# PKU-VCL-Geometry/GeoSplatting

Measured on AMD Instinct MI355X. Metric: fwd+bwd views/sec at 2M Gaussians, 800x800, higher is better.
Workload: dtype f32

## Files before the change

geosplatting_amd/csrc/gs_front.hip:

```cpp
#include "gs_common.h"
#include <string.h>
#pragma clang fp contract(off)
#include "gs_project_dev.h"
#include "gs_shade_dev.h"

template <int CTRL, int ROW_MASK>
__device__ __forceinline__ unsigned dpp_max_u32(unsigned v)
{
    const unsigned o = (unsigned)__builtin_amdgcn_update_dpp(0, (int)v, CTRL, ROW_MASK, 0xf, false);
    return o > v ? o : v;
}
__device__ __forceinline__ unsigned wave_max_u32_lane63(unsigned v)
{
    v = dpp_max_u32<0xB1, 0xf>(v);
    v = dpp_max_u32<0x4E, 0xf>(v);
    v = dpp_max_u32<0x141, 0xf>(v);
    v = dpp_max_u32<0x140, 0xf>(v);
    v = dpp_max_u32<0x142, 0xa>(v);
    v = dpp_max_u32<0x143, 0xc>(v);
    return v;
}

__global__ void __launch_bounds__(GS_PROJ_BLOCK)
front_fwd_kernel(int N, const float* __restrict__ means, const float* __restrict__ quats, const float* __restrict__ scales,
                 const float* __restrict__ opacities, const float* __restrict__ normals, const float* __restrict__ kd,
                 const float* __restrict__ ks, const float* __restrict__ viewmat, const float* __restrict__ K,
                 const float* __restrict__ cam_pos, float min_roughness, float max_metallic, int mode, EnvDev env,
                 int W, int H, int tile_size, int tile_w, int tile_h, float eps2d, float near_plane, float far_plane, float radius_clip,
                 unsigned key_base, unsigned key_limit , float4* __restrict__ vis, unsigned* __restrict__ depth_keys,
                 uint2* __restrict__ rects, unsigned* __restrict__ ctrl, u64* __restrict__ desc, int n_chunks,
                 unsigned long long* __restrict__ counts , long long* __restrict__ status,
                 unsigned* __restrict__ tile_counts , int32_t* __restrict__ packed_index ,
                 int tight_tiles)
{
    extern __shared__ unsigned s_th[];
    const int n_tiles = tile_w * tile_h;
    if (tile_counts) for (int t = threadIdx.x; t < n_tiles; t += GS_PROJ_BLOCK) s_th[t] = 0u;
    __shared__ int s_chunk;
    __shared__ int s_wv[GS_PROJ_WAVES];
    __shared__ int s_wi[GS_PROJ_WAVES];
    __shared__ unsigned s_wmx[GS_PROJ_WAVES], s_wmn[GS_PROJ_WAVES];
    __shared__ long long s_base[2];

    const int tid = threadIdx.x, lane = tid & 63, wave = tid >> 6;
    if (tid == 0) s_chunk = (int)atomicAdd(ctrl, 1u);
    __syncthreads();
    const int chunk = s_chunk;
    const int n = chunk * GS_PROJ_BLOCK + tid;

    u64* agg_v = desc;
    u64* agg_i = desc + n_chunks;
    u64* pre_v = desc + 2 * (size_t)n_chunks;
    u64* pre_i = desc + 3 * (size_t)n_chunks;

    const GsCam cam = load_cam(viewmat, K);
    ProjFwd p;
    p.valid = false; p.radius = 0;
    int ntiles = 0;
    int tx0 = 0, ty0 = 0, tx1 = 0, ty1 = 0;
    float mean[3] = { 0.f, 0.f, 0.f };
    float op = 0.0f, hx = -1.0f, hy = -1.0f;
    if (n < N) {
        mean[0] = means[3 * (size_t)n]; mean[1] = means[3 * (size_t)n + 1]; mean[2] = means[3 * (size_t)n + 2];
        const float4 q = *reinterpret_cast<const float4*>(quats + 4 * (size_t)n);
        const float quat[4] = { q.x, q.y, q.z, q.w };
        const float scale[3] = { scales[3 * (size_t)n], scales[3 * (size_t)n + 1], scales[3 * (size_t)n + 2] };
        p = project_exact(cam, mean, quat, scale, (float)W, (float)H, eps2d, near_plane, far_plane, radius_clip);
        if (p.valid) {
            tile_range_exact(p.m2x, p.m2y, p.radius, tile_size, tile_w, tile_h, tx0, ty0, tx1, ty1);
            op = opacities[n] * p.comp;
            if (!alpha_extent(p.ca, p.cb, p.cc, op, hx, hy)) { hx = -1.0f; hy = -1.0f; }
            if (tight_tiles) {
                if (hx < 0.0f) { tx1 = tx0; ty1 = ty0; }
                else {
                    const float ts = (float)tile_size;
                    const float fx0 = floorf((p.m2x - hx) / ts), fy0 = floorf((p.m2y - hy) / ts);
                    const float fx1 = ceilf((p.m2x + hx) / ts), fy1 = ceilf((p.m2y + hy) / ts);
                    const int ax0 = fx0 < 0.0f ? 0 : (fx0 > (float)tile_w ? tile_w : (int)fx0), ax1 = fx1 < 0.0f ? 0 : (fx1 > (float)tile_w ? tile_w : (int)fx1);
                    const int ay0 = fy0 < 0.0f ? 0 : (fy0 > (float)tile_h ? tile_h : (int)fy0), ay1 = fy1 < 0.0f ? 0 : (fy1 > (float)tile_h ? tile_h : (int)fy1);
                    tx0 = max(tx0, ax0); tx1 = min(tx1, ax1); ty0 = max(ty0, ay0); ty1 = min(ty1, ay1);
                    if (tx1 < tx0) tx1 = tx0;
                    if (ty1 < ty0) ty1 = ty0;
                }
            }
            ntiles = (tx1 - tx0) * (ty1 - ty0);
        }
    }

    const u64 bal = __ballot(p.valid);
    const int v_excl_wave = __popcll(bal & ((1ull << lane) - 1ull));
    int i_incl = ntiles;
    i_incl = gs_wave_incl_scan(i_incl);
    const unsigned dbits = p.valid ? __float_as_uint(p.depth) : 0u;
    {
        const unsigned mx = wave_max_u32_lane63(dbits), mn = wave_max_u32_lane63(p.valid ? ~dbits : 0u);
        if (lane == 63) { s_wv[wave] = __popcll(bal); s_wi[wave] = i_incl; s_wmx[wave] = mx; s_wmn[wave] = mn; }
    }
    __syncthreads();
    int v_before = 0, i_before = 0, aggV = 0, aggI = 0;
#pragma unroll
    for (int w = 0; w < GS_PROJ_WAVES; ++w) {
        if (w < wave) { v_before += s_wv[w]; i_before += s_wi[w]; }
        aggV += s_wv[w]; aggI += s_wi[w];
    }
    if (wave == 0 && lane == 0 && chunk > 0) { desc_store(&agg_v[chunk], (u64)aggV); desc_store(&agg_i[chunk], (u64)aggI); }

    const bool range_wave = wave == GS_PROJ_WAVES - 1;
    unsigned long long cur_mx = 0ull, cur_mn = 0ull;
    if (range_wave && lane == 0 && aggV != 0) {
        cur_mx = __hip_atomic_load(counts + 3, __ATOMIC_RELAXED, __HIP_MEMORY_SCOPE_AGENT);
        cur_mn = __hip_atomic_load(counts + 2, __ATOMIC_RELAXED, __HIP_MEMORY_SCOPE_AGENT);
    }

    float color[3] = { 0.f, 0.f, 0.f };
    if (p.valid && vis != nullptr) {
        const float nrm[3] = { normals[3 * (size_t)n], normals[3 * (size_t)n + 1], normals[3 * (size_t)n + 2] };
        const float kdn[3] = { kd[3 * (size_t)n], kd[3 * (size_t)n + 1], kd[3 * (size_t)n + 2] };
        const float2 ks2 = *reinterpret_cast<const float2*>(ks + 2 * (size_t)n);
        const float ksn[2] = { ks2.x, ks2.y };
        const float cp[3] = { cam_pos[0], cam_pos[1], cam_pos[2] };
        ShadeTmp t;
        shade_one<false>(mean, nrm, kdn, ksn, cp, min_roughness, max_metallic, mode, env, color, t);
    }
    if (range_wave && lane == 0 && aggV != 0) {
        unsigned mx = 0u, mn = 0u;
#pragma unroll
        for (int w = 0; w < GS_PROJ_WAVES; ++w) { mx = s_wmx[w] > mx ? s_wmx[w] : mx; mn = s_wmn[w] > mn ? s_wmn[w] : mn; }
        if ((unsigned long long)mx > cur_mx) atomicMax(counts + 3, (unsigned long long)mx);
        if ((unsigned long long)mn > cur_mn) atomicMax(counts + 2, (unsigned long long)mn);
    }
    unsigned key = dbits;
    if (key_limit != 0u) {
        const bool fits = dbits >= key_base && (dbits - key_base) < key_limit;
        if (p.valid && !fits && status) status[3] = 1;
        key = fits ? dbits - key_base : (dbits < key_base ? 0u : key_limit - 1u);
    }

    if (wave == 0) {
        long long baseV = 0, baseI = 0;
        if (chunk > 0) {
            int pos = chunk - 1;
            for (;;) {
                const int idx = pos - lane;
                bool isP = idx < 0;
                bool isA = false;
                u64 pv = 0, pi = 0, av = 0, ai = 0;
                if (idx >= 0) {
                    int spins = 0;
                    for (;;) {
                        pv = desc_load(&pre_v[idx]); pi = desc_load(&pre_i[idx]);
                        isP = (pv & pi & GS_VALID_BIT) != 0;
                        if (isP) break;
                        av = desc_load(&agg_v[idx]); ai = desc_load(&agg_i[idx]);
                        isA = (av & ai & GS_VALID_BIT) != 0;
                        if (isA) break;
                        if (++spins > GS_SPIN_LIMIT) {
                            atomicExch(ctrl + 1, 1u);
                            if (status) status[0] = GS_ENOSPC;
                            isA = true; av = ai = 0; break;
                        }
                        __builtin_amdgcn_s_sleep(2);
                    }
                }
                const u64 pmask = __ballot(isP);
                const int first = pmask ? __builtin_ctzll(pmask) : 64;
                long long cv = 0, ci = 0;
                if (lane <= first) {
                    cv = (long long)((isP ? pv : av) & ~GS_VALID_BIT);
                    ci = (long long)((isP ? pi : ai) & ~GS_VALID_BIT);
                }
                baseV += wave_sum_i64(cv);
                baseI += wave_sum_i64(ci);
                if (pmask) break;
                pos -= 64;
            }
        }
        if (lane == 0) {
            desc_store(&pre_i[chunk], (u64)(baseI + aggI));
            desc_store(&pre_v[chunk], (u64)(baseV + aggV));
            s_base[0] = baseV; s_base[1] = baseI;
            if (chunk == n_chunks - 1) { counts[0] = (unsigned long long)(baseV + aggV); counts[1] = (unsigned long long)(baseI + aggI); }
        }
    }
    __syncthreads();
    if (packed_index && n < N) packed_index[n] = p.valid ? (int32_t)(s_base[0] + v_before + v_excl_wave) : -1;
    if (p.valid) {
        const long long slot = s_base[0] + v_before + v_excl_wave;
        if (vis != nullptr) {
            float4* rec = vis + 4 * slot;
            rec[0] = make_float4(p.m2x, p.m2y, 0.5f * p.ca, p.cb);
            rec[1] = make_float4(0.5f * p.cc, op, hx, hy);
            rec[2] = make_float4(color[0], color[1], color[2], 0.0f);
            rec[3] = make_float4(p.comp, __int_as_float(n), p.depth, __int_as_float(p.radius));
        }
        if (depth_keys != nullptr) {
            depth_keys[slot] = key;
            rects[slot] = make_uint2((unsigned)tx0 | ((unsigned)ty0 << 16), (unsigned)tx1 | ((unsigned)ty1 << 16));
        }
        if (tile_counts)
            for (int i = ty0; i < ty1; ++i)
                for (int j = tx0; j < tx1; ++j) atomicAdd(&s_th[i * tile_w + j], 1u);
    }
    if (tile_counts) {
        __syncthreads();
        for (int t = threadIdx.x; t < n_tiles; t += GS_PROJ_BLOCK) { const unsigned c = s_th[t]; if (c) atomicAdd(tile_counts + t, c); }
    }
}

__global__ void __launch_bounds__(256)
front_setup_kernel(unsigned* __restrict__ ws, int ws_words, unsigned long long* __restrict__ counts4, unsigned* __restrict__ tile_counts, int n_tiles)
{
    const int i = blockIdx.x * blockDim.x + threadIdx.x, stride = gridDim.x * blockDim.x;
    for (int k = i; k < ws_words; k += stride) ws[k] = 0u;
    for (int k = i; k < n_tiles; k += stride) tile_counts[k] = 0u;
    if (i < 4) counts4[i] = 0ull;
}

#define GS_FRONT_HIST_MAX 8192
extern "C" size_t gs_front_ws_bytes(int N) { return (gs_project_ws_bytes(N) + 15) & ~(size_t)15; }

extern "C" int gs_front_fwd(int N, const float* means, const float* quats, const float* scales, const float* opacities,
                            const float* normals, const float* kd, const float* ks, const float* viewmat, const float* K,
                            const float* cam_pos, float min_roughness, float max_metallic, int mode, const GsEnv* env,
                            int W, int H, int tile_size, float eps2d, float near_plane, float far_plane, float radius_clip,
                            uint32_t key_base, int key_bits, float* vis_records, uint32_t* depth_keys, uint32_t* tile_rects,
                            uint32_t* tile_counts, int32_t* packed_index, int tight_tiles, int64_t* counts4, int64_t* status4, void* ws,
                            size_t ws_bytes, void* stream)
{
    GS_CHECK_ARG(N >= 0 && W > 0 && H > 0 && tile_size > 0 && mode >= 0 && mode <= 2, "bad sizes or mode");
    GS_CHECK_ARG(counts4 != nullptr && ws != nullptr, "null argument");
    GS_CHECK_ARG((depth_keys != nullptr) == (tile_rects != nullptr) && (vis_records != nullptr || depth_keys != nullptr),
                 "depth_keys and tile_rects go together; at least one of {vis_records} / {depth_keys, tile_rects} is wanted");
    GS_CHECK_ARG(key_bits == 24 || key_bits == 32, "key_bits must be 24 or 32");
    GS_CHECK_ARG(key_bits == 32 || status4 != nullptr, "24-bit keys need a status word (range overflow is reported there)");
    EnvDev e;
    if (vis_records != nullptr) GS_CHECK_ARG(env_to_dev(env, e) == 0, "bad GsEnv");
    else memset(&e, 0, sizeof(e));
    if (ws_bytes < gs_front_ws_bytes(N)) { gs_set_error("gs_front_fwd: workspace too small"); return GS_ENOSPC; }
    hipStream_t s = (hipStream_t)stream;
    const int tile_w = (W + tile_size - 1) / tile_size, tile_h = (H + tile_size - 1) / tile_size;
    GS_CHECK_ARG(tile_w < 65536 && tile_h < 65536, "tile grid too large");
    const int n_tiles = tile_w * tile_h;
    const bool hist = tile_counts != nullptr && n_tiles <= GS_FRONT_HIST_MAX;
    const int ws_words = (int)(gs_front_ws_bytes(N) / 4);
    hipLaunchKernelGGL(front_setup_kernel, dim3(gs_cdiv(ws_words > n_tiles ? ws_words : n_tiles, 256) < 64 ? gs_cdiv(ws_words > n_tiles ? ws_words : n_tiles, 256) : 64),
                       dim3(256), 0, s, (unsigned*)ws, ws_words, (unsigned long long*)counts4, tile_counts, tile_counts ? n_tiles : 0);
    GS_CHECK_LAUNCH();
    if (N == 0) return GS_OK;
    const int n_chunks = (N + GS_PROJ_BLOCK - 1) / GS_PROJ_BLOCK;
    hipLaunchKernelGGL(front_fwd_kernel, dim3(n_chunks), dim3(GS_PROJ_BLOCK), hist ? (size_t)n_tiles * sizeof(unsigned) : 0, s, N, means, quats, scales, opacities, normals, kd, ks,
                       viewmat, K, cam_pos, min_roughness, max_metallic, mode, e, W, H, tile_size, tile_w, tile_h, eps2d, near_plane,
                       far_plane, radius_clip, key_bits == 24 ? key_base : 0u, key_bits == 24 ? (1u << 24) : 0u, (float4*)vis_records,
                       depth_keys, (uint2*)tile_rects, (unsigned*)ws, (u64*)((char*)ws + 16), n_chunks, (unsigned long long*)counts4,
                       (long long*)status4, hist ? tile_counts : (unsigned*)nullptr, packed_index, tight_tiles);
    GS_CHECK_LAUNCH();
    return GS_OK;
}

template <int BLOCK>
__global__ void __launch_bounds__(BLOCK)
tail_bwd_kernel(GsCount vc, const float* __restrict__ means, const float* __restrict__ quats, const float* __restrict__ scales,
                const float* __restrict__ opacities, const float* __restrict__ normals, const float* __restrict__ kd,
                const float* __restrict__ ks, const float* __restrict__ viewmat, const float* __restrict__ K,
                const float* __restrict__ cam_pos, float min_roughness, float max_metallic, int mode, EnvDev env, int W, int H,
                float eps2d, const float4* __restrict__ vis, const float* __restrict__ v_packed, int rec_stride,
                float* __restrict__ v_means, float* __restrict__ v_quats, float* __restrict__ v_scales, float* __restrict__ v_opacities,
                float* __restrict__ v_normals, float* __restrict__ v_kd, float* __restrict__ v_ks, EnvGradDev eg)
{
    extern __shared__ __attribute__((aligned(16))) float s_grad[];
    for (int i = threadIdx.x; i < eg.lds_floats; i += blockDim.x) s_grad[i] = 0.0f;
    __syncthreads();
    float* const stage = s_grad + eg.stage_off + (threadIdx.x >> 6) * 640;
    float* const priv = eg.priv ? eg.priv + (long long)gs_xcc_id() * eg.priv_stride : nullptr;
    const float cp[3] = { cam_pos[0], cam_pos[1], cam_pos[2] };
    const GsCam cam = load_cam(viewmat, K);
    const int V = (int)gs_count(vc);
    const int stride = (int)(gridDim.x * blockDim.x);
    const int n_iter = (V + stride - 1) / stride;
    for (int it = 0; it < n_iter; ++it) {
        const int v = it * stride + blockIdx.x * blockDim.x + threadIdx.x;
        bool scatter = false;
        ShadeTmp t;
        float v_ls[3] = { 0, 0, 0 }, v_ld[3] = { 0, 0, 0 };
        if (v < V) {
            const float4 r0 = vis[4 * (size_t)v], r1 = vis[4 * (size_t)v + 1], r3 = vis[4 * (size_t)v + 3];
            const int n = __float_as_int(r3.y);
            const float4* gp = reinterpret_cast<const float4*>(v_packed + (size_t)v * rec_stride);
            const float4 g0 = gp[0], g1 = gp[1];
            const float g2 = v_packed[(size_t)v * rec_stride + 8];
            const float g[3] = { g1.z, g1.w, g2 };
            const bool any_geo = g0.x != 0.0f || g0.y != 0.0f || g0.z != 0.0f || g0.w != 0.0f || g1.x != 0.0f || g1.y != 0.0f;
            const bool any_col = g[0] != 0.0f || g[1] != 0.0f || g[2] != 0.0f;
            if (any_geo || any_col) {
                const float mean[3] = { means[3 * (size_t)n], means[3 * (size_t)n + 1], means[3 * (size_t)n + 2] };
                float o_mean[3] = { 0, 0, 0 };
                if (any_geo) {
                    const float4 q4 = *reinterpret_cast<const float4*>(quats + 4 * (size_t)n);
                    const float scale[3] = { scales[3 * (size_t)n], scales[3 * (size_t)n + 1], scales[3 * (size_t)n + 2] };
                    ProjGrad pg;
                    project_bwd_one(cam, mean, q4, scale, opacities[n], (float)W, (float)H, eps2d, 2.0f * r0.z, r0.w, 2.0f * r1.x, r3.x,
                                    g0.x, g0.y, g0.z, g0.w, g1.x, g1.y, 0.0f, pg);
                    float4 q = *reinterpret_cast<float4*>(v_quats + 4 * (size_t)n);
                    q.x += pg.quat[0]; q.y += pg.quat[1]; q.z += pg.quat[2]; q.w += pg.quat[3];
                    *reinterpret_cast<float4*>(v_quats + 4 * (size_t)n) = q;
#pragma unroll
                    for (int k = 0; k < 3; ++k) { v_scales[3 * (size_t)n + k] += pg.scale[k]; o_mean[k] = pg.mean[k]; }
                    v_opacities[n] += pg.op;
                }
                if (any_col) {
                    const float normal[3] = { normals[3 * (size_t)n], normals[3 * (size_t)n + 1], normals[3 * (size_t)n + 2] };
                    const float kdn[3] = { kd[3 * (size_t)n], kd[3 * (size_t)n + 1], kd[3 * (size_t)n + 2] };
                    const float2 ks2 = *reinterpret_cast<const float2*>(ks + 2 * (size_t)n);
                    const float ksn[2] = { ks2.x, ks2.y };
                    float color[3];
                    shade_one<true>(mean, normal, kdn, ksn, cp, min_roughness, max_metallic, mode, env, color, t);
                    scatter = true;
                    float v_diff[3] = { 0, 0, 0 }, v_rf[3] = { 0, 0, 0 };
#pragma unroll
                    for (int c = 0; c < 3; ++c) {
                        if (mode == GS_MODE_PBR)          { v_diff[c] = g[c]; v_ls[c] = g[c] * t.refl_c[c]; v_rf[c] = g[c] * t.ls.out[c]; }
                        else if (mode == GS_MODE_DIFFUSE) { v_ld[c] = g[c] * t.diff[c]; v_diff[c] = g[c] * t.ld[c]; }
                        else                              { v_ls[c] = g[c] * t.refl_c[c]; v_rf[c] = g[c] * t.ls.out[c]; }
                    }
                    float v_A = 0.0f, v_B = 0.0f, v_metal = 0.0f, o_kd[3];
#pragma unroll
                    for (int c = 0; c < 3; ++c) {
                        const float v_spec = v_rf[c] * t.fg[0];
                        v_A += v_rf[c] * t.spec[c];
                        v_B += v_rf[c];
                        o_kd[c] = v_spec * t.metal + v_diff[c] * (1.0f - t.metal);
                        v_metal += v_spec * (kdn[c] - 0.04f) - v_diff[c] * kdn[c];
                    }
                    const float v_ndv = v_A * t.dfg_du[0] + v_B * t.dfg_du[1];
                    float v_rough = v_A * t.dfg_dv[0] + v_B * t.dfg_dv[1];
                    float v_mip = 0.0f, v_refl[3] = { 0, 0, 0 }, v_n[3] = { 0, 0, 0 };
                    if (mode != GS_MODE_DIFFUSE) {
#pragma unroll
                        for (int c = 0; c < 3; ++c) {
                            v_mip += v_ls[c] * t.ls.dmip[c];
#pragma unroll
                            for (int k = 0; k < 3; ++k) v_refl[k] += v_ls[c] * t.ls.dd[c * 3 + k];
                        }
                    } else {
#pragma unroll
                        for (int c = 0; c < 3; ++c)
#pragma unroll
                            for (int k = 0; k < 3; ++k) v_n[k] += v_ld[c] * t.ld_dd[c * 3 + k];
                    }
                    v_rough += v_mip * t.dmip_dr;
                    float v_d = 2.0f * (v_refl[0] * normal[0] + v_refl[1] * normal[1] + v_refl[2] * normal[2]);
                    float v_wo[3];
#pragma unroll
                    for (int k = 0; k < 3; ++k) { v_n[k] += 2.0f * t.d * v_refl[k]; v_wo[k] = -v_refl[k]; }
                    if (t.d >= 1e-6f) v_d += v_ndv;
#pragma unroll
                    for (int k = 0; k < 3; ++k) { v_n[k] += v_d * t.wo[k]; v_wo[k] += v_d * normal[k]; }
                    if (!t.wo_const) {
                        const float dot = t.wo[0] * v_wo[0] + t.wo[1] * v_wo[1] + t.wo[2] * v_wo[2];
                        const float l = fmaxf(t.len, 1e-6f);
#pragma unroll
                        for (int k = 0; k < 3; ++k) o_mean[k] += -((v_wo[k] - t.wo[k] * dot) / l);
                    }
#pragma unroll
                    for (int k = 0; k < 3; ++k) { v_normals[3 * (size_t)n + k] += v_n[k]; v_kd[3 * (size_t)n + k] += o_kd[k]; }
                    float2 o = *reinterpret_cast<float2*>(v_ks + 2 * (size_t)n);
                    o.x += v_rough * (1.0f - min_roughness); o.y += v_metal * max_metallic;
                    *reinterpret_cast<float2*>(v_ks + 2 * (size_t)n) = o;
                }
#pragma unroll
                for (int k = 0; k < 3; ++k) v_means[3 * (size_t)n + k] += o_mean[k];
            }
        }
        if (mode != GS_MODE_DIFFUSE) {
            const int l0 = scatter ? t.ls.l0 : 0, l1 = scatter ? t.ls.l1 : -1;
            const float w0 = (l1 < 0) ? 1.0f : 1.0f - t.ls.f;
            const bool lds0 = scatter && eg.lds_level[l0] >= 0;
            if (lds0) cube_scatter_lds(s_grad + eg.lds_level[l0], t.ls.fp0, v_ls, w0);
            const bool loc0 = priv != nullptr && eg.priv_level[l0] >= 0;
            cube_scatter_wave_tagged(scatter && !lds0 ? (loc0 ? priv + eg.priv_level[l0] : eg.levels[l0]) : nullptr, loc0, t.ls.fp0, v_ls, w0,
                                     scatter && !lds0, stage);
            const bool has1 = scatter && l1 >= 0;
            const int l1s = has1 ? l1 : 0;
            const bool lds1 = has1 && eg.lds_level[l1s] >= 0;
            if (lds1) cube_scatter_lds(s_grad + eg.lds_level[l1], t.ls.fp1, v_ls, t.ls.f);
            const bool loc1 = priv != nullptr && eg.priv_level[l1s] >= 0;
            cube_scatter_wave_tagged(has1 && !lds1 ? (loc1 ? priv + eg.priv_level[l1s] : eg.levels[l1s]) : nullptr, loc1, t.ls.fp1, v_ls, t.ls.f,
                                     has1 && !lds1, stage);
        } else {
            const bool ldsb = scatter && eg.lds_base >= 0;
            if (ldsb) cube_scatter_lds(s_grad + eg.lds_base, t.ld_fp, v_ld, 1.0f);
            cube_scatter_wave_tagged(scatter && !ldsb ? eg.base : nullptr, false, t.ld_fp, v_ld, 1.0f, scatter && !ldsb, stage);
        }
    }
    __syncthreads();
    if (eg.lds_base >= 0) {
        const int cnt = 18 * env.base_res * env.base_res;
        for (int i = threadIdx.x; i < cnt; i += blockDim.x) {
            const float x = s_grad[eg.lds_base + i];
            if (x != 0.0f) gs_atomic_add(eg.base + i, x);
        }
    }
    for (int l = 0; l < env.L; ++l) {
        if (eg.lds_level[l] < 0) continue;
        const int cnt = 18 * env.res[l] * env.res[l];
        for (int i = threadIdx.x; i < cnt; i += blockDim.x) {
            const float x = s_grad[eg.lds_level[l] + i];
            if (x != 0.0f) gs_atomic_add(eg.levels[l] + i, x);
        }
    }
}

static int tail_background_blocks() { return 128; }
static int tail_priv_maxres() { return 128; }
static size_t tail_priv_floats(const EnvDev& e, int mode, long long* level_off)
{
    long long off = 0;
    for (int l = 0; l < GS_MAX_LEVELS; ++l) level_off[l] = -1;
    if (mode != GS_MODE_DIFFUSE)
        for (int l = 0; l < e.L; ++l)
            if (e.res[l] > 32 && e.res[l] <= tail_priv_maxres()) { level_off[l] = off; off += 18ll * e.res[l] * e.res[l]; }
    return (size_t)((off + 63) / 64 * 64);
}

extern "C" size_t gs_tail_priv_ws_bytes(const GsEnv* env, int mode)
{
    EnvDev e;
    if (env_to_dev(env, e) != 0) return 0;
    long long lo[GS_MAX_LEVELS];
    return tail_priv_floats(e, mode, lo) * sizeof(float) * GS_XCD_COPIES;
}

extern "C" int gs_tail_priv_reduce(const GsEnv* env, int mode, const void* priv_ws, size_t priv_ws_bytes, const GsEnvGrad* env_grad, void* stream)
{
    EnvDev e;
    GS_CHECK_ARG(env_to_dev(env, e) == 0 && env_grad != nullptr, "bad GsEnv / env_grad");
    long long lo[GS_MAX_LEVELS];
    const size_t floats = tail_priv_floats(e, mode, lo);
    if (floats == 0 || priv_ws == nullptr) return GS_OK;
    if (priv_ws_bytes < floats * sizeof(float) * GS_XCD_COPIES) { gs_set_error("gs_tail_priv_reduce: workspace too small"); return GS_ENOSPC; }
    for (int l = 0; l < e.L; ++l) {
        if (lo[l] < 0) continue;
        GS_CHECK_ARG(env_grad->levels[l] != nullptr, "env_grad->levels[l] required");
        const long long n = 18ll * e.res[l] * e.res[l];
        hipLaunchKernelGGL(priv_reduce_kernel, dim3((int)((n + 255) / 256 < 2048 ? (n + 255) / 256 : 2048)), dim3(256), 0, (hipStream_t)stream, n,
                           GS_XCD_COPIES, (const float*)priv_ws + lo[l], (long long)floats, env_grad->levels[l]);
        GS_CHECK_LAUNCH();
    }
    return GS_OK;
}

extern "C" int gs_tail_bwd(int V_cap, const int64_t* counts_dev , const float* means, const float* quats,
                           const float* scales, const float* opacities, const float* normals, const float* kd, const float* ks,
                           const float* viewmat, const float* K, const float* cam_pos, float min_roughness, float max_metallic, int mode,
                           const GsEnv* env, int W, int H, float eps2d, const float* vis_records, const float* v_packed, int rec_stride,
                           float* v_means, float* v_quats, float* v_scales, float* v_opacities, float* v_normals, float* v_kd, float* v_ks,
                           const GsEnvGrad* env_grad, void* priv_ws, size_t priv_ws_bytes, void* stream)
{
    GS_CHECK_ARG(V_cap >= 0 && mode >= 0 && mode <= 2 && rec_stride >= 12 && (rec_stride % 4) == 0, "bad sizes, mode or record stride");
    EnvDev e;
    GS_CHECK_ARG(env_to_dev(env, e) == 0, "bad GsEnv");
    GS_CHECK_ARG(env_grad != nullptr && vis_records != nullptr && v_packed != nullptr, "null argument");
    EnvGradDev eg;
    eg.base = env_grad->base;
    for (int l = 0; l < GS_MAX_LEVELS; ++l) eg.levels[l] = l < e.L ? env_grad->levels[l] : nullptr;
    if (mode == GS_MODE_DIFFUSE) GS_CHECK_ARG(eg.base != nullptr, "env_grad->base required in diffuse mode");
    else for (int l = 0; l < e.L; ++l) GS_CHECK_ARG(eg.levels[l] != nullptr, "env_grad->levels[l] required");
    ShadeBwdPlan plan;
    { const int rc = shade_bwd_plan(e, mode, V_cap, nullptr, 0, eg, plan, true); if (rc != GS_OK) return rc; }
    {
        const size_t floats = tail_priv_floats(e, mode, eg.priv_level);
        if (priv_ws != nullptr && floats > 0) {
            if (priv_ws_bytes < floats * sizeof(float) * GS_XCD_COPIES) { gs_set_error("gs_tail_bwd: private workspace too small"); return GS_ENOSPC; }
            eg.priv = (float*)priv_ws; eg.priv_stride = (long long)floats;
        } else {
            eg.priv = nullptr; eg.priv_stride = 0;
            for (int l = 0; l < GS_MAX_LEVELS; ++l) eg.priv_level[l] = -1;
        }
    }
    if (V_cap == 0) return GS_OK;
    hipStream_t s = (hipStream_t)stream;
    const GsCount vc{ (long long)V_cap, (const long long*)counts_dev };
#define GS_TAIL_LAUNCH(B)                                                                                                              \
    do {                                                                                                                               \
        GS_CHECK_HIP(hipFuncSetAttribute((const void*)tail_bwd_kernel<B>, hipFuncAttributeMaxDynamicSharedMemorySize, (int)plan.lds_bytes)); \
        hipLaunchKernelGGL((tail_bwd_kernel<B>), dim3(plan.blocks), dim3(B), plan.lds_bytes, s, vc, means, quats, scales, opacities, normals, \
                           kd, ks, viewmat, K, cam_pos, min_roughness, max_metallic, mode, e, W, H, eps2d, (const float4*)vis_records,   \
                           v_packed, rec_stride, v_means, v_quats, v_scales, v_opacities, v_normals, v_kd, v_ks, eg);                    \
        GS_CHECK_LAUNCH();                                                                                                             \
    } while (0)
    if (plan.block == 1024) GS_TAIL_LAUNCH(1024); else if (plan.block == 768) GS_TAIL_LAUNCH(768); else if (plan.block == 256) GS_TAIL_LAUNCH(256);
    else GS_TAIL_LAUNCH(512);
#undef GS_TAIL_LAUNCH
    return GS_OK;
}


#define GS_TAIL_MAX_VIEWS 8
struct TailViewDev {
    const float* viewmat; const float* K; const float* cam_pos;
    const float4* vis; const float* v_packed; const int32_t* packed_index;
    int W, H;
};
struct TailViewsDev { TailViewDev v[GS_TAIL_MAX_VIEWS]; int n; };

#define GS_TAILP_BLOCK 1024
struct TailViewLds {
    unsigned long long vis, v_packed, packed_index;
    float cam[16];
    float cam_pos[3];
    float Wf, Hf;
    float pad;
};

struct TailLevelLds { unsigned long long tex, gtex; long long priv_off; int R, lds_off; };

template <int VPG>
__device__ __forceinline__ float tail_group_sum(float v)
{
    if (VPG >= 2) v = gs_dpp_add<0xB1, 0xf, 0xf>(v);
    if (VPG >= 4) v = gs_dpp_add<0x4E, 0xf, 0xf>(v);
    if (VPG >= 8) v = gs_dpp_add<0x141, 0xf, 0xf>(v);
    return v;
}

template <int BLOCK, int VPG>
__global__ void __launch_bounds__(BLOCK)
tail_proj_pairs_kernel(int N, TailViewsDev views, const float* __restrict__ means, const float* __restrict__ quats,
                       const float* __restrict__ scales, const float* __restrict__ opacities, float eps2d, int rec_stride,
                       float* __restrict__ v_means, float* __restrict__ v_quats, float* __restrict__ v_scales,
                       float* __restrict__ v_opacities, int accumulate)
{
    __shared__ TailViewLds s_views[VPG];
#pragma unroll
    for (int k = 0; k < VPG; ++k) {
        if ((int)threadIdx.x == k) {
            const TailViewDev& h = views.v[k];
            TailViewLds& d = s_views[k];
            d.vis = (unsigned long long)h.vis; d.v_packed = (unsigned long long)h.v_packed; d.packed_index = (unsigned long long)h.packed_index;
            const GsCam c = load_cam(h.viewmat, h.K);
#pragma unroll
            for (int i = 0; i < 9; ++i) d.cam[i] = c.R[i];
            d.cam[9] = c.t[0]; d.cam[10] = c.t[1]; d.cam[11] = c.t[2];
            d.cam[12] = c.fx; d.cam[13] = c.fy; d.cam[14] = c.cx; d.cam[15] = c.cy;
            d.cam_pos[0] = d.cam_pos[1] = d.cam_pos[2] = 0.0f;
            d.Wf = (float)h.W; d.Hf = (float)h.H; d.pad = 0.0f;
        }
    }
    __syncthreads();
    constexpr int G = BLOCK / VPG;
    const int view = (int)threadIdx.x & (VPG - 1), gl = (int)threadIdx.x / VPG;
    const TailViewLds& vw = s_views[view];
    const int n = (int)blockIdx.x * G + gl;
    const bool live = n < N && view < views.n;
// ... 342 lines not shown
```

Measured before the change: 725.1.

## Process two Gaussians per thread in fused front projection kernel

New measurement: 739.9, median of 6. 2.1% higher.

```diff
diff --git a/geosplatting_amd/csrc/gs_front.hip b/geosplatting_amd/csrc/gs_front.hip
--- a/geosplatting_amd/csrc/gs_front.hip
+++ b/geosplatting_amd/csrc/gs_front.hip
@@ -21,7 +21,13 @@
     return v;
 }
 
-__global__ void __launch_bounds__(GS_PROJ_BLOCK)
+#define GS_FRONT_BLOCK 256
+#define GS_FRONT_ITEMS 2
+#define GS_FRONT_WAVES (GS_FRONT_BLOCK / 64)
+#define GS_FRONT_CHUNK (GS_FRONT_BLOCK * GS_FRONT_ITEMS)
+#define GS_FRONT_PARTS (GS_FRONT_ITEMS * GS_FRONT_WAVES)
+
+__global__ void __launch_bounds__(GS_FRONT_BLOCK) __attribute__((amdgpu_waves_per_eu(4)))
 front_fwd_kernel(int N, const float* __restrict__ means, const float* __restrict__ quats, const float* __restrict__ scales,
                  const float* __restrict__ opacities, const float* __restrict__ normals, const float* __restrict__ kd,
                  const float* __restrict__ ks, const float* __restrict__ viewmat, const float* __restrict__ K,
@@ -35,18 +41,18 @@
 {
     extern __shared__ unsigned s_th[];
     const int n_tiles = tile_w * tile_h;
-    if (tile_counts) for (int t = threadIdx.x; t < n_tiles; t += GS_PROJ_BLOCK) s_th[t] = 0u;
+    if (tile_counts) for (int t = threadIdx.x; t < n_tiles; t += GS_FRONT_BLOCK) s_th[t] = 0u;
     __shared__ int s_chunk;
-    __shared__ int s_wv[GS_PROJ_WAVES];
-    __shared__ int s_wi[GS_PROJ_WAVES];
-    __shared__ unsigned s_wmx[GS_PROJ_WAVES], s_wmn[GS_PROJ_WAVES];
+    __shared__ int s_wv[GS_FRONT_PARTS];
+    __shared__ int s_wi[GS_FRONT_PARTS];
+    __shared__ unsigned s_wmx[GS_FRONT_WAVES], s_wmn[GS_FRONT_WAVES];
     __shared__ long long s_base[2];
 
     const int tid = threadIdx.x, lane = tid & 63, wave = tid >> 6;
     if (tid == 0) s_chunk = (int)atomicAdd(ctrl, 1u);
     __syncthreads();
     const int chunk = s_chunk;
-    const int n = chunk * GS_PROJ_BLOCK + tid;
+    const int n0 = chunk * GS_FRONT_CHUNK + tid;
 
     u64* agg_v = desc;
     u64* agg_i = desc + n_chunks;
@@ -54,28 +60,41 @@
     u64* pre_i = desc + 3 * (size_t)n_chunks;
 
     const GsCam cam = load_cam(viewmat, K);
-    ProjFwd p;
-    p.valid = false; p.radius = 0;
-    int ntiles = 0;
-    int tx0 = 0, ty0 = 0, tx1 = 0, ty1 = 0;
-    float mean[3] = { 0.f, 0.f, 0.f };
-    float op = 0.0f, hx = -1.0f, hy = -1.0f;
-    if (n < N) {
-        mean[0] = means[3 * (size_t)n]; mean[1] = means[3 * (size_t)n + 1]; mean[2] = means[3 * (size_t)n + 2];
-        const float4 q = *reinterpret_cast<const float4*>(quats + 4 * (size_t)n);
-        const float quat[4] = { q.x, q.y, q.z, q.w };
-        const float scale[3] = { scales[3 * (size_t)n], scales[3 * (size_t)n + 1], scales[3 * (size_t)n + 2] };
-        p = project_exact(cam, mean, quat, scale, (float)W, (float)H, eps2d, near_plane, far_plane, radius_clip);
-        if (p.valid) {
-            tile_range_exact(p.m2x, p.m2y, p.radius, tile_size, tile_w, tile_h, tx0, ty0, tx1, ty1);
-            op = opacities[n] * p.comp;
-            if (!alpha_extent(p.ca, p.cb, p.cc, op, hx, hy)) { hx = -1.0f; hy = -1.0f; }
+
+    float mean[GS_FRONT_ITEMS][3], scale[GS_FRONT_ITEMS][3], opac[GS_FRONT_ITEMS];
+    float4 qv[GS_FRONT_ITEMS];
+#pragma unroll
+    for (int k = 0; k < GS_FRONT_ITEMS; ++k) {
+        const int n = n0 + k * GS_FRONT_BLOCK;
+        const size_t nn = (size_t)(n < N ? n : N - 1);
+        mean[k][0] = means[3 * nn]; mean[k][1] = means[3 * nn + 1]; mean[k][2] = means[3 * nn + 2];
+        qv[k] = *reinterpret_cast<const float4*>(quats + 4 * nn);
+        scale[k][0] = scales[3 * nn]; scale[k][1] = scales[3 * nn + 1]; scale[k][2] = scales[3 * nn + 2];
+        opac[k] = opacities[nn];
+    }
+
+    ProjFwd p[GS_FRONT_ITEMS];
+    int ntiles[GS_FRONT_ITEMS];
+    unsigned rect0[GS_FRONT_ITEMS], rect1[GS_FRONT_ITEMS];
+    float op[GS_FRONT_ITEMS], hx[GS_FRONT_ITEMS], hy[GS_FRONT_ITEMS];
+#pragma unroll
+    for (int k = 0; k < GS_FRONT_ITEMS; ++k) {
+        const int n = n0 + k * GS_FRONT_BLOCK;
+        const float quat[4] = { qv[k].x, qv[k].y, qv[k].z, qv[k].w };
+        p[k] = project_exact(cam, mean[k], quat, scale[k], (float)W, (float)H, eps2d, near_plane, far_plane, radius_clip);
+        if (n >= N) { p[k].valid = false; p[k].radius = 0; }
+        int tx0 = 0, ty0 = 0, tx1 = 0, ty1 = 0;
+        ntiles[k] = 0; op[k] = 0.0f; hx[k] = -1.0f; hy[k] = -1.0f;
+        if (p[k].valid) {
+            tile_range_exact(p[k].m2x, p[k].m2y, p[k].radius, tile_size, tile_w, tile_h, tx0, ty0, tx1, ty1);
+            op[k] = opac[k] * p[k].comp;
+            if (!alpha_extent(p[k].ca, p[k].cb, p[k].cc, op[k], hx[k], hy[k])) { hx[k] = -1.0f; hy[k] = -1.0f; }
             if (tight_tiles) {
-                if (hx < 0.0f) { tx1 = tx0; ty1 = ty0; }
+                if (hx[k] < 0.0f) { tx1 = tx0; ty1 = ty0; }
                 else {
                     const float ts = (float)tile_size;
-                    const float fx0 = floorf((p.m2x - hx) / ts), fy0 = floorf((p.m2y - hy) / ts);
-                    const float fx1 = ceilf((p.m2x + hx) / ts), fy1 = ceilf((p.m2y + hy) / ts);
+                    const float fx0 = floorf((p[k].m2x - hx[k]) / ts), fy0 = floorf((p[k].m2y - hy[k]) / ts);
+                    const float fx1 = ceilf((p[k].m2x + hx[k]) / ts), fy1 = ceilf((p[k].m2y + hy[k]) / ts);
                     const int ax0 = fx0 < 0.0f ? 0 : (fx0 > (float)tile_w ? tile_w : (int)fx0), ax1 = fx1 < 0.0f ? 0 : (fx1 > (float)tile_w ? tile_w : (int)fx1);
                     const int ay0 = fy0 < 0.0f ? 0 : (fy0 > (float)tile_h ? tile_h : (int)fy0), ay1 = fy1 < 0.0f ? 0 : (fy1 > (float)tile_h ? tile_h : (int)fy1);
                     tx0 = max(tx0, ax0); tx1 = min(tx1, ax1); ty0 = max(ty0, ay0); ty1 = min(ty1, ay1);
@@ -83,57 +102,91 @@
                     if (ty1 < ty0) ty1 = ty0;
                 }
             }
-            ntiles = (tx1 - tx0) * (ty1 - ty0);
-        }
-    }
-
-    const u64 bal = __ballot(p.valid);
-    const int v_excl_wave = __popcll(bal & ((1ull << lane) - 1ull));
-    int i_incl = ntiles;
-    i_incl = gs_wave_incl_scan(i_incl);
-    const unsigned dbits = p.valid ? __float_as_uint(p.depth) : 0u;
+            ntiles[k] = (tx1 - tx0) * (ty1 - ty0);
+        }
+        rect0[k] = (unsigned)tx0 | ((unsigned)ty0 << 16);
+        rect1[k] = (unsigned)tx1 | ((unsigned)ty1 << 16);
+    }
+
+    int v_excl_wave[GS_FRONT_ITEMS];
+    unsigned dbits[GS_FRONT_ITEMS];
+    bool any_valid = false;
     {
-        const unsigned mx = wave_max_u32_lane63(dbits), mn = wave_max_u32_lane63(p.valid ? ~dbits : 0u);
-        if (lane == 63) { s_wv[wave] = __popcll(bal); s_wi[wave] = i_incl; s_wmx[wave] = mx; s_wmn[wave] = mn; }
+        unsigned dmx = 0u, dmn = 0u;
+#pragma unroll
+        for (int k = 0; k < GS_FRONT_ITEMS; ++k) {
+            const u64 bal = __ballot(p[k].valid);
+            v_excl_wave[k] = __popcll(bal & ((1ull << lane) - 1ull));
+            const int i_incl = gs_wave_incl_scan(ntiles[k]);
+            if (lane == 63) { s_wv[k * GS_FRONT_WAVES + wave] = __popcll(bal); s_wi[k * GS_FRONT_WAVES + wave] = i_incl; }
+            dbits[k] = p[k].valid ? __float_as_uint(p[k].depth) : 0u;
+            const unsigned nb = p[k].valid ? ~dbits[k] : 0u;
+            dmx = dbits[k] > dmx ? dbits[k] : dmx; dmn = nb > dmn ? nb : dmn;
+            any_valid = any_valid || p[k].valid;
+        }
+        const unsigned mx = wave_max_u32_lane63(dmx), mn = wave_max_u32_lane63(dmn);
+        if (lane == 63) { s_wmx[wave] = mx; s_wmn[wave] = mn; }
     }
     __syncthreads();
-    int v_before = 0, i_before = 0, aggV = 0, aggI = 0;
-#pragma unroll
-    for (int w = 0; w < GS_PROJ_WAVES; ++w) {
-        if (w < wave) { v_before += s_wv[w]; i_before += s_wi[w]; }
-        aggV += s_wv[w]; aggI += s_wi[w];
+    int aggV = 0, aggI = 0;
+#pragma unroll
+    for (int k = 0; k < GS_FRONT_ITEMS; ++k) {
+#pragma unroll
+        for (int w = 0; w < GS_FRONT_WAVES; ++w) {
+            if (w == wave) v_excl_wave[k] += aggV;
+            aggV += s_wv[k * GS_FRONT_WAVES + w]; aggI += s_wi[k * GS_FRONT_WAVES + w];
+        }
     }
     if (wave == 0 && lane == 0 && chunk > 0) { desc_store(&agg_v[chunk], (u64)aggV); desc_store(&agg_i[chunk], (u64)aggI); }
 
-    const bool range_wave = wave == GS_PROJ_WAVES - 1;
+    const bool range_wave = wave == GS_FRONT_WAVES - 1;
     unsigned long long cur_mx = 0ull, cur_mn = 0ull;
     if (range_wave && lane == 0 && aggV != 0) {
         cur_mx = __hip_atomic_load(counts + 3, __ATOMIC_RELAXED, __HIP_MEMORY_SCOPE_AGENT);
         cur_mn = __hip_atomic_load(counts + 2, __ATOMIC_RELAXED, __HIP_MEMORY_SCOPE_AGENT);
     }
 
-    float color[3] = { 0.f, 0.f, 0.f };
-    if (p.valid && vis != nullptr) {
-        const float nrm[3] = { normals[3 * (size_t)n], normals[3 * (size_t)n + 1], normals[3 * (size_t)n + 2] };
-        const float kdn[3] = { kd[3 * (size_t)n], kd[3 * (size_t)n + 1], kd[3 * (size_t)n + 2] };
-        const float2 ks2 = *reinterpret_cast<const float2*>(ks + 2 * (size_t)n);
-        const float ksn[2] = { ks2.x, ks2.y };
+    float color[GS_FRONT_ITEMS][3];
+#pragma unroll
+    for (int k = 0; k < GS_FRONT_ITEMS; ++k) { color[k][0] = 0.f; color[k][1] = 0.f; color[k][2] = 0.f; }
+    if (any_valid && vis != nullptr) {
+        float nrm[GS_FRONT_ITEMS][3], kdn[GS_FRONT_ITEMS][3], ksn[GS_FRONT_ITEMS][2];
+#pragma unroll
+        for (int k = 0; k < GS_FRONT_ITEMS; ++k) {
+            const int n = n0 + k * GS_FRONT_BLOCK;
+            const size_t nn = (size_t)(n < N ? n : N - 1);
+            nrm[k][0] = normals[3 * nn]; nrm[k][1] = normals[3 * nn + 1]; nrm[k][2] = normals[3 * nn + 2];
+            kdn[k][0] = kd[3 * nn]; kdn[k][1] = kd[3 * nn + 1]; kdn[k][2] = kd[3 * nn + 2];
+            const float2 ks2 = *reinterpret_cast<const float2*>(ks + 2 * nn);
+            ksn[k][0] = ks2.x; ksn[k][1] = ks2.y;
+        }
         const float cp[3] = { cam_pos[0], cam_pos[1], cam_pos[2] };
-        ShadeTmp t;
-        shade_one<false>(mean, nrm, kdn, ksn, cp, min_roughness, max_metallic, mode, env, color, t);
+#pragma unroll
+        for (int k = 0; k < GS_FRONT_ITEMS; ++k) {
+            ShadeTmp t;
+            shade_one<false>(mean[k], nrm[k], kdn[k], ksn[k], cp, min_roughness, max_metallic, mode, env, color[k], t);
+        }
     }
     if (range_wave && lane == 0 && aggV != 0) {
         unsigned mx = 0u, mn = 0u;
 #pragma unroll
-        for (int w = 0; w < GS_PROJ_WAVES; ++w) { mx = s_wmx[w] > mx ? s_wmx[w] : mx; mn = s_wmn[w] > mn ? s_wmn[w] : mn; }
+        for (int w = 0; w < GS_FRONT_WAVES; ++w) { mx = s_wmx[w] > mx ? s_wmx[w] : mx; mn = s_wmn[w] > mn ? s_wmn[w] : mn; }
         if ((unsigned long long)mx > cur_mx) atomicMax(counts + 3, (unsigned long long)mx);
         if ((unsigned long long)mn > cur_mn) atomicMax(counts + 2, (unsigned long long)mn);
     }
-    unsigned key = dbits;
-    if (key_limit != 0u) {
-        const bool fits = dbits >= key_base && (dbits - key_base) < key_limit;
-        if (p.valid && !fits && status) status[3] = 1;
-        key = fits ? dbits - key_base : (dbits < key_base ? 0u : key_limit - 1u);
+    unsigned key[GS_FRONT_ITEMS];
+    {
+        bool outside = false;
+#pragma unroll
+        for (int k = 0; k < GS_FRONT_ITEMS; ++k) {
+            key[k] = dbits[k];
+            if (key_limit != 0u) {
+                const bool fits = dbits[k] >= key_base && (dbits[k] - key_base) < key_limit;
+                outside = outside || (p[k].valid && !fits);
+                key[k] = fits ? dbits[k] - key_base : (dbits[k] < key_base ? 0u : key_limit - 1u);
+            }
+        }
+        if (outside && status) status[3] = 1;
     }
 
     if (wave == 0) {
@@ -183,27 +236,34 @@
         }
     }
     __syncthreads();
-    if (packed_index && n < N) packed_index[n] = p.valid ? (int32_t)(s_base[0] + v_before + v_excl_wave) : -1;
-    if (p.valid) {
-        const long long slot = s_base[0] + v_before + v_excl_wave;
-        if (vis != nullptr) {
-            float4* rec = vis + 4 * slot;
-            rec[0] = make_float4(p.m2x, p.m2y, 0.5f * p.ca, p.cb);
-            rec[1] = make_float4(0.5f * p.cc, op, hx, hy);
-            rec[2] = make_float4(color[0], color[1], color[2], 0.0f);
-            rec[3] = make_float4(p.comp, __int_as_float(n), p.depth, __int_as_float(p.radius));
-        }
-        if (depth_keys != nullptr) {
-            depth_keys[slot] = key;
-            rects[slot] = make_uint2((unsigned)tx0 | ((unsigned)ty0 << 16), (unsigned)tx1 | ((unsigned)ty1 << 16));
-        }
-        if (tile_counts)
-            for (int i = ty0; i < ty1; ++i)
-                for (int j = tx0; j < tx1; ++j) atomicAdd(&s_th[i * tile_w + j], 1u);
+    const long long slot_base = s_base[0];
+#pragma unroll
+    for (int k = 0; k < GS_FRONT_ITEMS; ++k) {
+        const int n = n0 + k * GS_FRONT_BLOCK;
+        const long long slot = slot_base + v_excl_wave[k];
+        if (packed_index && n < N) packed_index[n] = p[k].valid ? (int32_t)slot : -1;
+        if (p[k].valid) {
+            if (vis != nullptr) {
+                float4* rec = vis + 4 * slot;
+                rec[0] = make_float4(p[k].m2x, p[k].m2y, 0.5f * p[k].ca, p[k].cb);
+                rec[1] = make_float4(0.5f * p[k].cc, op[k], hx[k], hy[k]);
+                rec[2] = make_float4(color[k][0], color[k][1], color[k][2], 0.0f);
+                rec[3] = make_float4(p[k].comp, __int_as_float(n), p[k].depth, __int_as_float(p[k].radius));
+            }
+            if (depth_keys != nullptr) {
+                depth_keys[slot] = key[k];
+                rects[slot] = make_uint2(rect0[k], rect1[k]);
+            }
+            if (tile_counts) {
+                const int tx0 = (int)(rect0[k] & 0xffffu), ty0 = (int)(rect0[k] >> 16), tx1 = (int)(rect1[k] & 0xffffu), ty1 = (int)(rect1[k] >> 16);
+                for (int i = ty0; i < ty1; ++i)
+                    for (int j = tx0; j < tx1; ++j) atomicAdd(&s_th[i * tile_w + j], 1u);
+            }
+        }
     }
     if (tile_counts) {
         __syncthreads();
-        for (int t = threadIdx.x; t < n_tiles; t += GS_PROJ_BLOCK) { const unsigned c = s_th[t]; if (c) atomicAdd(tile_counts + t, c); }
+        for (int t = threadIdx.x; t < n_tiles; t += GS_FRONT_BLOCK) { const unsigned c = s_th[t]; if (c) atomicAdd(tile_counts + t, c); }
     }
 }
 
@@ -217,7 +277,8 @@
 }
 
 #define GS_FRONT_HIST_MAX 8192
-extern "C" size_t gs_front_ws_bytes(int N) { return (gs_project_ws_bytes(N) + 15) & ~(size_t)15; }
+static int front_chunks(int N) { return N > 0 ? (N + GS_FRONT_CHUNK - 1) / GS_FRONT_CHUNK : 1; }
+extern "C" size_t gs_front_ws_bytes(int N) { return (16 + 4 * (size_t)front_chunks(N) * sizeof(u64) + 15) & ~(size_t)15; }
 
 extern "C" int gs_front_fwd(int N, const float* means, const float* quats, const float* scales, const float* opacities,
                             const float* normals, const float* kd, const float* ks, const float* viewmat, const float* K,
@@ -247,8 +308,8 @@
                        dim3(256), 0, s, (unsigned*)ws, ws_words, (unsigned long long*)counts4, tile_counts, tile_counts ? n_tiles : 0);
     GS_CHECK_LAUNCH();
     if (N == 0) return GS_OK;
-    const int n_chunks = (N + GS_PROJ_BLOCK - 1) / GS_PROJ_BLOCK;
-    hipLaunchKernelGGL(front_fwd_kernel, dim3(n_chunks), dim3(GS_PROJ_BLOCK), hist ? (size_t)n_tiles * sizeof(unsigned) : 0, s, N, means, quats, scales, opacities, normals, kd, ks,
+    const int n_chunks = front_chunks(N);
+    hipLaunchKernelGGL(front_fwd_kernel, dim3(n_chunks), dim3(GS_FRONT_BLOCK), hist ? (size_t)n_tiles * sizeof(unsigned) : 0, s, N, means, quats, scales, opacities, normals, kd, ks,
                        viewmat, K, cam_pos, min_roughness, max_metallic, mode, e, W, H, tile_size, tile_w, tile_h, eps2d, near_plane,
                        far_plane, radius_clip, key_bits == 24 ? key_base : 0u, key_bits == 24 ? (1u << 24) : 0u, (float4*)vis_records,
                        depth_keys, (uint2*)tile_rects, (unsigned*)ws, (u64*)((char*)ws + 16), n_chunks, (unsigned long long*)counts4,
```
